# cczls1991/DL_Biomass

Measured on NVIDIA B200. Metric: train tree-clouds/sec @10k pts, higher is better.
Workload: dtype bf16

## Files before the change

### dl_biomass_b200/_lib.py

```python
from __future__ import annotations

import ctypes
import os
import shutil
import subprocess

_HERE = os.path.dirname(os.path.abspath(__file__))
LIB_PATH = os.path.join(_HERE, "libb2pn.so")
CSRC = os.path.join(_HERE, "csrc")

_lib = None
ABI_VERSION = 7

_vp, _i32, _i64, _f32, _f64 = ctypes.c_void_p, ctypes.c_int32, ctypes.c_int64, ctypes.c_float, ctypes.c_double

class Mlp3(ctypes.Structure):
    _fields_ = [("c", ctypes.c_int32 * 4), ("act", ctypes.c_int32), ("eps", ctypes.c_float),
                ("momentum", ctypes.c_float), ("w", _vp * 3), ("b", _vp * 3), ("gamma", _vp * 2),
                ("beta", _vp * 2), ("running_mean", _vp * 2), ("running_var", _vp * 2),
                ("num_batches_tracked", _vp * 2)]


class SaArgs(ctypes.Structure):
    _fields_ = [("precision", ctypes.c_int32), ("training", ctypes.c_int32), ("seg_mode", ctypes.c_int32),
                ("K", ctypes.c_int32), ("n_src", ctypes.c_int64), ("n_dst", ctypes.c_int64),
                ("c_in", ctypes.c_int32), ("x_dtype", ctypes.c_int32), ("x", _vp), ("pos_src", _vp),
                ("pos_dst", _vp), ("nbr", _vp), ("cnt", _vp), ("batch", _vp), ("mlp", Mlp3), ("out", _vp),
                ("arg", _vp), ("h1", _vp), ("h2", _vp), ("bn", _vp), ("workspace", _vp),
                ("workspace_bytes", ctypes.c_int64), ("rgrp", _vp), ("row_src", _vp), ("num_rows", _vp),
                ("row_capacity", ctypes.c_int64), ("row_valid", _vp), ("a1", _vp), ("a2", _vp), ("g1", _vp),
                ("g1_ready", ctypes.c_int32), ("sm_limit", ctypes.c_int32), ("deterministic", ctypes.c_int32),
                ("out_bf16", _vp)]


class FpsOptions(ctypes.Structure):
    _fields_ = [("cluster", ctypes.c_int32), ("threads", ctypes.c_int32), ("seed", ctypes.c_uint64), ("rng_state", _vp)]


class SaGrads(ctypes.Structure):
    _fields_ = [("grad_out", _vp), ("grad_w", _vp * 3), ("grad_b", _vp * 3), ("grad_gamma", _vp * 2),
                ("grad_beta", _vp * 2), ("grad_x", _vp)]

class AugmentCloud(ctypes.Structure):
    _fields_ = [("src_off", ctypes.c_int64), ("out_off", ctypes.c_int64), ("uid", ctypes.c_uint64),
                ("n_src", ctypes.c_int32), ("n_keep", ctypes.c_int32), ("n_dup", ctypes.c_int32),
                ("noise_sd", ctypes.c_float), ("cos_a", ctypes.c_float), ("sin_a", ctypes.c_float)]

# ... 81 lines not shown
```

### dl_biomass_b200/csrc/sa_chain.cuh

```cuda
#pragma once

namespace b2pn {
namespace tc {

constexpr int CH_ROWS = 64;
constexpr int CH_SLOTS = 2;
constexpr int CH_EPI_WARPS = 8;
constexpr int CH_EPI_THREADS = CH_EPI_WARPS * 32;
constexpr int CH_LOAD_THREADS = 128;
constexpr int CH_MMA_WARP = CH_SLOTS * CH_EPI_WARPS;
constexpr int CH_THREADS = CH_SLOTS * CH_EPI_THREADS + CH_SLOTS * 32 + CH_SLOTS * CH_LOAD_THREADS;
constexpr int CH_CHUNK_BYTES = CH_ROWS * LINE_BYTES;
constexpr int CH_TMEM_PER_SLOT = 256;

struct ChainParams {
    const uint8_t *w_img[3];
    int w_bytes[3];
    int k_img;
    int k1c, c1c, c2c;
    int c1, c2, c3;
    int mt3;
    int64_t rows;
    const int64_t *rows_dev;
    const float *bias[3];
// ... 288 lines not shown
                        }
                    }
                }
            }
            tc_fence_before();
            __syncwarp();
            if (lane == 0) mbar_arrive(&b[CB_D3_FREE]);
        }
    }
    tc_fence_before();
    __syncthreads();
    if (warp == CH_MMA_WARP) tmem_dealloc<512>(tmem_base);
}

constexpr int CT_THREADS = CH_SLOTS * CH_EPI_THREADS + CH_SLOTS * 32 + CH_SLOTS * 32;
enum { TB_IN_FULL = 0, TB_IN_FREE, TB_DA_FULL, TB_XA_FULL, TB_DB_FULL, TB_DB_FREE, TB_PER_SLOT };

struct ChainTrainParams {
    const uint8_t *w_img[2];
    int w_bytes[2];
    int k_in;
    int kc_in, kc_mid;
    int c_a, c_b;
    int mt_b;
    int64_t rows;
    const int64_t *rows_dev;
    int64_t ld;
    const float *bias_a, *mean_a, *rstd_a, *gamma_a, *beta_a;
    int dup_a;
    int act;
    __half *z_out, *a_out;
    double *partial;
    int cpad;
    const float *bias_b;
    float *out;
    int32_t *arg;
    __half *out16;
    const uint32_t *rgrp;
};

template <int PASS, int KCI_, int NKSL_, int KCM_, int MTB_>
__global__ void __launch_bounds__(CT_THREADS, 1)
    tc_chain_train_kernel(const ChainTrainParams p, const __grid_constant__ TmaMap map_in, const __grid_constant__ TmaMap map_z,
                          const __grid_constant__ TmaMap map_a)
{
    static_assert(PASS == 2 || PASS == 3, "PASS 2: layer 1 + statistics of layer 2; PASS 3: layer 2 + layer 3 + max");
    const int kc_in = KCI_ >= 0 ? KCI_ : p.kc_in;
    const int kc_mid = KCM_ >= 0 ? KCM_ : p.kc_mid;
    const int mt_b = MTB_ >= 0 ? MTB_ : p.mt_b;
    const int nks_last = NKSL_ >= 0 ? NKSL_ : ((p.k_in - (p.kc_in - 1) * KC) >= KC ? 4 : (p.k_in - (p.kc_in - 1) * KC + 15) / 16);
    extern __shared__ uint8_t smem_raw[];
    uint8_t *smem = reinterpret_cast<uint8_t *>((reinterpret_cast<uintptr_t>(smem_raw) + 1023) & ~(uintptr_t)1023);
    uint8_t *Wa = smem, *Wb = Wa + p.w_bytes[0];
    uint8_t *slots = Wb + p.w_bytes[1];
    const int in_bytes = kc_in * CH_CHUNK_BYTES, x_bytes = kc_mid * CH_CHUNK_BYTES;
    const int slot_bytes = in_bytes + 2 * x_bytes;
    uint64_t *bars = reinterpret_cast<uint64_t *>(slots + CH_SLOTS * slot_bytes);
    uint64_t *w_full = bars + CH_SLOTS * TB_PER_SLOT;
    uint32_t *tmem_holder = reinterpret_cast<uint32_t *>(w_full + 1);

    const int tid = threadIdx.x, warp = tid >> 5, lane = tid & 31;
    const int64_t rows = p.rows_dev ? *p.rows_dev : p.rows;
    const int64_t num_tiles = ((rows + 127) / 128) * 2;

    if (tid == 0) {
        for (int s = 0; s < CH_SLOTS; ++s) {
            uint64_t *b = bars + s * TB_PER_SLOT;
            mbar_init(&b[TB_IN_FULL], 1);
            mbar_init(&b[TB_IN_FREE], 1);
            mbar_init(&b[TB_DA_FULL], 1);
            mbar_init(&b[TB_XA_FULL], 1);
            mbar_init(&b[TB_DB_FULL], 1);
            mbar_init(&b[TB_DB_FREE], CH_EPI_WARPS);
        }
        mbar_init(w_full, 1);
        fence_barrier_init();
    }
    if (warp == CH_MMA_WARP) tmem_alloc<512>(tmem_holder);
    tc_fence_before();
    __syncthreads();
    tc_fence_after();
    const uint32_t tmem_base = *tmem_holder;
    auto tile_of = [&](int64_t it, int s) { return (it * (int64_t)gridDim.x + blockIdx.x) * CH_SLOTS + s; };
    unsigned leader;
    asm volatile("{\n\t.reg .pred p;\n\telect.sync _|p, 0xffffffff;\n\tselp.u32 %0, 1, 0, p;\n\t}" : "=r"(leader));

    if (warp >= CH_MMA_WARP + CH_SLOTS) {
        const int s = warp - (CH_MMA_WARP + CH_SLOTS);
        if (s < CH_SLOTS && leader) {
            uint64_t *b = bars + s * TB_PER_SLOT;
            uint8_t *IN = slots + s * slot_bytes;
            for (int64_t it = 0;; ++it) {
                const int64_t tile = tile_of(it, s);
                if (tile >= num_tiles) break;
                mbar_wait(&b[TB_IN_FREE], (uint32_t)(it & 1) ^ 1u);
                mbar_expect_tx(&b[TB_IN_FULL], (unsigned)in_bytes);
                for (int kc = 0; kc < kc_in; ++kc)
                    tma_load_2d(IN + kc * CH_CHUNK_BYTES, &map_in, (int)(tile * CH_ROWS), kc * KC, &b[TB_IN_FULL]);
                mbar_arrive(&b[TB_IN_FULL]);
            }
        }
    } else if (warp >= CH_MMA_WARP) {
        const int s = warp - CH_MMA_WARP;
        if (s == 0 && leader) {
            mbar_expect_tx(w_full, (unsigned)(p.w_bytes[0] + p.w_bytes[1]));
            for (int l = 0; l < 2; ++l) {
                uint8_t *dst = l == 0 ? Wa : Wb;
                for (int off = 0; off < p.w_bytes[l]; off += 16384) bulk_g2s(dst + off, p.w_img[l] + off, 16384u, w_full);
            }
            mbar_arrive(w_full);
        }
        __syncwarp();
        mbar_wait(w_full, 0);
        const uint32_t idesc_mn = idesc_16(128, CH_ROWS, false, true, FMT_F16, FMT_F16);
        uint64_t *b = bars + s * TB_PER_SLOT;
        uint8_t *IN = slots + s * slot_bytes;
        const uint64_t dwa = smem_desc_sw128(smem_u32(Wa), 16, ATOM_BYTES);
        const uint64_t dwb = smem_desc_sw128(smem_u32(Wb), 16, ATOM_BYTES);
        const uint64_t din = smem_desc_sw128(smem_u32(IN), 64 * LINE_BYTES, ATOM_BYTES);
        const uint64_t dx = smem_desc_sw128(smem_u32(IN + in_bytes), 64 * LINE_BYTES, ATOM_BYTES);
        constexpr uint64_t A_KS = 32 >> 4, A_CHUNK = (128 * LINE_BYTES) >> 4, B_KS_MN = (16 * LINE_BYTES) >> 4,
                           B_CHUNK = CH_CHUNK_BYTES >> 4;
        const uint32_t da = tmem_base + s * CH_TMEM_PER_SLOT, db = da + 64;
        for (int64_t it = 0;; ++it) {
            if (tile_of(it, s) >= num_tiles) break;
            const uint32_t ph = (uint32_t)(it & 1);
            mbar_wait(&b[TB_IN_FULL], ph);
            tc_fence_after();
            if (leader) {
#pragma unroll
                for (int kc = 0; kc < (KCI_ >= 0 ? KCI_ : 3); ++kc) {
                    if (kc < kc_in) {
#pragma unroll
                        for (int ks = 0; ks < 4; ++ks)
                            if (kc + 1 < kc_in || ks < nks_last)
                                umma_bf16(da, dwa + kc * A_CHUNK + ks * A_KS, din + kc * B_CHUNK + ks * B_KS_MN, idesc_mn, (kc | ks) != 0);
                    }
                }
                umma_commit(&b[TB_IN_FREE]);
                umma_commit(&b[TB_DA_FULL]);
            }
            __syncwarp();
            mbar_wait(&b[TB_XA_FULL], ph);
            mbar_wait(&b[TB_DB_FREE], ph ^ 1u);
            tc_fence_after();
            if (leader) {
#pragma unroll
                for (int mt = 0; mt < (MTB_ >= 0 ? MTB_ : 2); ++mt) {
                    if (mt < mt_b) {
#pragma unroll
                        for (int kc = 0; kc < (KCM_ >= 0 ? KCM_ : 2); ++kc) {
                            if (kc < kc_mid) {
#pragma unroll
                                for (int ks = 0; ks < 4; ++ks)
                                    umma_bf16(db + mt * 64, dwb + (uint64_t)(kc * mt_b + mt) * A_CHUNK + ks * A_KS,
                                              dx + kc * B_CHUNK + ks * B_KS_MN, idesc_mn, (kc | ks) != 0);
                            }
                        }
                    }
                }
                umma_commit(&b[TB_DB_FULL]);
            }
            __syncwarp();
        }
    } else {
        const int s = warp / CH_EPI_WARPS, w8 = warp % CH_EPI_WARPS;
        const int q = w8 & 3, half = w8 >> 2;
        uint64_t *b = bars + s * TB_PER_SLOT;
        uint8_t *X = slots + s * slot_bytes + in_bytes;
        const int ch = q * 32 + lane;
        const uint32_t lane_addr = ((uint32_t)(q * 32)) << 16;
        const uint32_t da = tmem_base + lane_addr + s * CH_TMEM_PER_SLOT, db = da + 64;
        const bool dup = (KCM_ == 1 || KCM_ < 0) && p.dup_a != 0;
        const int cha = dup ? (q & 1) * 32 + lane : ch;
        const int col16 = half * 2 + (q >> 1);
        float sc = 0.f, sh = 0.f, ga = 0.f, be = 0.f;
        if (cha < p.c_a) {
            sc = p.rstd_a[cha];
            sh = (p.bias_a[cha] - p.mean_a[cha]) * sc;
            ga = p.gamma_a[cha];
            be = p.beta_a[cha];
        }
        const bool relu = p.act == B2PN_ACT_RELU;
        const int chb = (PASS == 3 && mt_b == 2 ? half * 128 : 0) + ch;
        const bool epb = PASS == 2 || mt_b == 2 || half == 0;
        const float bb = (PASS == 3 && epb && chb < p.c_b) ? p.bias_b[chb] : 0.f;
        uint8_t *xline = X + (cha >> 6) * CH_CHUNK_BYTES + (cha & 63) * LINE_BYTES;
        const int sw = cha & 7;
// ... 8 lines not shown
            const int64_t tile = tile_of(it, s);
            if (tile >= num_tiles) break;
            const uint32_t ph = (uint32_t)(it & 1);
            const int64_t row0 = tile * CH_ROWS;
            unsigned dsc[8] = {nx0.x, nx0.y, nx0.z, nx0.w, nx1.x, nx1.y, nx1.z, nx1.w};
#pragma unroll
            for (int g = 0; g < 8; ++g) {
                const int64_t gi = tile * (CH_ROWS / 8) + g;
                if (gi * 8 >= rows || gi_none(dsc[g])) dsc[g] = GI_NONE;
            }
            if (tile_of(it + 1, s) < num_tiles) {
                const uint4 *t = reinterpret_cast<const uint4 *>(p.rgrp + tile_of(it + 1, s) * (CH_ROWS / 8));
                nx0 = __ldg(t);
                nx1 = __ldg(t + 1);
            }
            mbar_wait(&b[TB_DA_FULL], ph);
            tc_fence_after();
            if (w8 == 0 && lane == 0) bulk_wait_read_all();
            asm volatile("bar.sync %0, %1;" ::"r"(1 + s), "n"(CH_EPI_THREADS) : "memory");
            if (dup) {
                unsigned nv2 = 0u;
#pragma unroll
                for (int g = 0; g < 8; ++g)
                    if ((g >> 1) == col16) nv2 |= (unsigned)gi_nv(dsc[g]) << (4 * (g & 1));
                float v[16];
                tmem_ld16(da + col16 * 16, v);
#pragma unroll
                for (int j = 0; j < 2; ++j) {
                    const int nv = (int)((nv2 >> (4 * j)) & 15u);
                    float f[8], g[8];
#pragma unroll
                    for (int e = 0; e < 8; ++e) f[e] = fmaf(v[8 * j + e], sc, sh);
                    const uint4 zq = pack8h(f);
                    unpack8h(zq, f);
#pragma unroll
                    for (int e = 0; e < 8; ++e) {
                        float y = fmaf(f[e], ga, be);
                        if (relu) y = fmaxf(y, 0.f);
                        g[e] = e < nv ? y : 0.f;
                    }
                    const int off = ((col16 * 2 + j) ^ sw) << 4;
                    *reinterpret_cast<uint4 *>(xline + x_bytes + off) = zq;
                    *reinterpret_cast<uint4 *>(xline + off) = pack8h(g);
                }
            } else if (ch - lane < p.c_a) {
                float v[32];
                tmem_ld32(da + half * 32, v);
#pragma unroll
                for (int j = 0; j < 4; ++j) {
                    const int nv = gi_nv(half == 0 ? dsc[j] : dsc[4 + j]);
                    float f[8], g[8];
#pragma unroll
                    for (int e = 0; e < 8; ++e) f[e] = fmaf(v[8 * j + e], sc, sh);
                    const uint4 zq = pack8h(f);
                    unpack8h(zq, f);
#pragma unroll
                    for (int e = 0; e < 8; ++e) {
                        float y = fmaf(f[e], ga, be);
                        if (relu) y = fmaxf(y, 0.f);
                        g[e] = e < nv ? y : 0.f;
                    }
                    const int off = ((half * 4 + j) ^ sw) << 4;
                    *reinterpret_cast<uint4 *>(xline + x_bytes + off) = zq;
                    *reinterpret_cast<uint4 *>(xline + off) = pack8h(g);
                }
            }
            fence_proxy_async_smem();
            tc_fence_before();
            asm volatile("bar.sync %0, %1;" ::"r"(1 + s), "n"(CH_EPI_THREADS) : "memory");
            if (w8 == 0 && lane == 0) {
                for (int kc = 0; kc < kc_mid; ++kc) {
                    tma_store_2d(&map_z, X + x_bytes + kc * CH_CHUNK_BYTES, (int)row0, kc * KC);
                    tma_store_2d(&map_a, X + kc * CH_CHUNK_BYTES, (int)row0, kc * KC);
                }
                bulk_commit_group();
                mbar_arrive(&b[TB_XA_FULL]);
            }
            mbar_wait(&b[TB_DB_FULL], ph);
            tc_fence_after();
            if (PASS == 2) {
                if (ch - lane < p.c_b) {
                    float v[32];
                    tmem_ld32(db + half * 32, v);
                    float sm = 0.f, qm = 0.f;
#pragma unroll
                    for (int j = 0; j < 32; ++j) {
                        sm += v[j];
                        qm = fmaf(v[j], v[j], qm);
                    }
                    S += (double)sm;
                    Q += (double)qm;
                }
            } else if (epb && chb - lane < p.c_b) {
                const uint32_t dcol = db + (mt_b == 2 ? half * 64 : 0);
                float best = -INFINITY;
                int bk = -1;
#pragma unroll 1
                for (int cc = 0; cc < 2; ++cc) {
                    float v[32];
                    tmem_ld32(dcol + cc * 32, v);
#pragma unroll
                    for (int gg = 0; gg < 4; ++gg) {
                        const unsigned inf = cc == 0 ? dsc[gg] : dsc[4 + gg];
                        if (gi_none(inf)) continue;
                        const int s0 = gi_slot0(inf), nv = gi_nv(inf);
                        if (s0 == 0) {
// ... 11 lines not shown
                        if (gi_last(inf) && chb < p.c_b) {
                            const int64_t m = gi_seg(inf);
                            const float o = bk >= 0 ? best : 0.f;
                            p.out[m * p.c_b + chb] = o;
                            p.arg[m * p.c_b + chb] = bk;
                            if (p.out16) p.out16[m * p.c_b + chb] = __float2half_rn(o);
                        }
                    }
                }
            }
            tc_fence_before();
            __syncwarp();
            if (lane == 0) mbar_arrive(&b[TB_DB_FREE]);
        }
        if (w8 == 0 && lane == 0) bulk_wait_all();
        if (PASS == 2 && ch < p.c_b) {
            double *pt = p.partial + ((int64_t)blockIdx.x * 4 + s * 2 + half) * 2 * p.cpad;
            pt[ch] = S;
            pt[p.cpad + ch] = Q;
        }
    }
    tc_fence_before();
    __syncthreads();
    if (warp == CH_MMA_WARP) tmem_dealloc<512>(tmem_base);
}

static int chain_train_smem_bytes(const ChainTrainParams &p)
{
    return p.w_bytes[0] + p.w_bytes[1] + CH_SLOTS * (p.kc_in + 2 * p.kc_mid) * CH_CHUNK_BYTES + 256 + 1024;
}

static bool chain_shapes_ok(const b2pn_sa_args &a, int k_lines, int c1, int c2, int c3)
{
    return a.seg_mode == B2PN_SEG_SLOTS && c1 % 64 == 0 && c2 % 64 == 0 && c1 <= 128 && c2 <= 128 && c3 <= 256 &&
           k_lines <= 3 * KC;
}

static int chain_smem_bytes(const ChainParams &p)
{
    const int x_bytes = (p.c1c > p.c2c ? p.c1c : p.c2c) * CH_CHUNK_BYTES;
    return p.w_bytes[0] + p.w_bytes[1] + p.w_bytes[2] + CH_SLOTS * (p.k1c * CH_CHUNK_BYTES + x_bytes) + 256 + 1024;
}

}
// ... 2 lines not shown
```

### dl_biomass_b200/csrc/sa_tc.cu

```cuda
#include <cuda.h>
#include <math.h>

#include "tc_common.cuh"

namespace b2pn {
namespace tc {

constexpr int R = 128;
constexpr int KC = 64;
constexpr int NUM_EPI = 256;
constexpr int NUM_LOAD = 128;
constexpr int LOAD_GROUPS = 2;
constexpr int MMA_WARP = (NUM_EPI + LOAD_GROUPS * NUM_LOAD) / 32;
constexpr int NT = NUM_EPI + LOAD_GROUPS * NUM_LOAD + 32;
constexpr int NT_TMA = 2 * NUM_EPI + 64;
constexpr int PROD_WARP_TMA = MMA_WARP + 1;
constexpr int NT_WIDE = 2 * NUM_EPI + 32 + NUM_LOAD;
constexpr int B_BYTES = R * LINE_BYTES;

constexpr unsigned GI_NONE = 0x00ffffffu;
__device__ __forceinline__ int gi_seg(unsigned b) { return (int)(b & 0xffffffu); }
__device__ __forceinline__ bool gi_none(unsigned b) { return (b & 0xffffffu) == 0xffffffu; }
__device__ __forceinline__ int gi_slot0(unsigned b) { return (int)((b >> 24) & 7u) << 3; }
__device__ __forceinline__ int gi_nv(unsigned b) { return (int)((b >> 27) & 15u); }
// ... 1992 lines not shown
    template <class T>
    T *take(int64_t n)
    {
        T *r = base ? (T *)(base + off) : nullptr;
        off = align_up(off + n * (int64_t)sizeof(T), 1024);
        return r;
    }
};

struct ShapesTC {
    int64_t rows, tiles, ld;
    int c0, c1, c2, c3, cmax, cpad, k1;
    InCols cols;
    int ctas;
    bool deterministic;
};
static ShapesTC shapes_tc(const b2pn_sa_args &a)
{
    ShapesTC s;
    s.rows = a.seg_mode == B2PN_SEG_CLOUDS ? a.n_src : a.row_capacity;
    s.tiles = (s.rows + R - 1) / R;
    s.ld = s.tiles * R;
    s.c0 = a.mlp.c[0];
    s.c1 = a.mlp.c[1];
    s.c2 = a.mlp.c[2];
    s.c3 = a.mlp.c[3];
    s.cmax = s.c1 > s.c2 ? s.c1 : s.c2;
    s.cols = InCols{a.c_in, a.x_dtype == B2PN_X_F32 ? 1 : 0};
    s.k1 = s.cols.k_img();
    int mx = s.cmax > s.c3 ? s.cmax : s.c3;
    mx = mx > s.k1 + 1 ? mx : s.k1 + 1;
    s.cpad = (int)align_up(mx, 128);
    s.ctas = cta_budget(a);
    s.deterministic = a.deterministic != 0;
    return s;
}

constexpr int MAX_GX = 160;

int sa_eval_fused_bf16(const b2pn_sa_args &a)
{
    if (a.mlp.c[0] != a.c_in + 3) return 0;
    const ShapesTC s = shapes_tc(a);
    return !a.training && chain_shapes_ok(a, s.k1, s.c1, s.c2, s.c3) ? 1 : 0;
}

static int check_args_tc(const b2pn_sa_args &a)
{
    if (a.n_src < 0 || a.n_dst < 0 || a.c_in < 0) return B2PN_EINVAL;
    if (a.mlp.c[0] != a.c_in + 3 || a.mlp.c[1] <= 0 || a.mlp.c[2] <= 0 || a.mlp.c[3] <= 0) return B2PN_EINVAL;
    if (a.mlp.act != B2PN_ACT_NONE && a.mlp.act != B2PN_ACT_RELU) return B2PN_ENOTSUP;
    if (a.x_dtype != B2PN_X_F32 && a.x_dtype != B2PN_X_BF16) return B2PN_EINVAL;
    if (a.seg_mode == B2PN_SEG_SLOTS) {
        if (a.K <= 0) return B2PN_EINVAL;
        if (a.K > 64) return B2PN_ENOTSUP;
        if (a.n_dst > 0 && (!a.nbr || !a.cnt || !a.pos_dst)) return B2PN_EINVAL;
        if (a.n_dst > 0 && (!a.rgrp || !a.row_src || !a.num_rows)) return B2PN_EINVAL;
        if (a.n_dst > 0 && a.row_capacity < b2pn_pack_rows_capacity(a.n_dst, a.K)) return B2PN_EINVAL;
    } else if (a.seg_mode == B2PN_SEG_CLOUDS) {
        if (a.n_src > 0 && !a.batch) return B2PN_EINVAL;
    } else {
        return B2PN_EINVAL;
    }
    if (a.n_src > 0 && (!a.pos_src || (a.c_in > 0 && !a.x))) return B2PN_EINVAL;
    for (int l = 0; l < 3; ++l)
        if (!a.mlp.w[l] || !a.mlp.b[l]) return B2PN_EINVAL;
    for (int l = 0; l < 2; ++l)
// ... 129 lines not shown
    B2PN_LAUNCH_CHECK();
    return B2PN_OK;
}

static void launch_bn_fwd_finalize(const b2pn_sa_args &a, const ShapesTC &s, int l, const double *partial, int nparts,
                                   const CountArg &count, cudaStream_t st)
{
    const int C = l == 0 ? s.c1 : s.c2;
    bn_fwd_finalize_tc_kernel<<<(C + 3) / 4, 128, 0, st>>>(partial, nparts, C, s.cpad, count, a.training, a.mlp.b[l], a.mlp.gamma[l],
                                                           a.mlp.beta[l], a.mlp.running_mean[l], a.mlp.running_var[l],
                                                           a.mlp.num_batches_tracked[l], a.mlp.eps, a.mlp.momentum,
                                                           a.bn + l * 4 * s.cmax, s.cmax);
    note_launch();
}

static int chain_grid(const ShapesTC &s, int64_t tiles64)
{
    const int64_t need = (tiles64 + CH_SLOTS - 1) / CH_SLOTS;
    return need < s.ctas ? (int)need : s.ctas;
}

template <auto KERN, class... Args>
static int launch_chain(int gx, int threads, int smem, cudaStream_t st, const Args &...args)
{
    static SmemAttrSlot slot = {};
    cudaError_t e = ensure_dynamic_smem(KERN, smem, slot);
    if (e != cudaSuccess) return (int)e;
    KERN<<<gx, threads, smem, st>>>(args...);
    note_launch();
    e = cudaPeekAtLastError();
    return e == cudaSuccess ? 0 : (int)e;
}

int sa_forward_bf16(const b2pn_sa_args &a, cudaStream_t st)
{
    int rc = check_args_tc(a);
    if (rc) return rc;
    const ShapesTC s = shapes_tc(a);
    if (a.n_dst == 0) return B2PN_OK;
    if (a.workspace_bytes < sa_workspace_bytes_bf16(a, 0) || !a.workspace) return B2PN_EINVAL;
    WsTC ws(a.workspace);
    FwdWsTC f = carve_fwd_tc(a, s, ws);
    const RowMapTC rm = rowmap_tc(a, s);
    const RowsArg ra = rowsarg_tc(a, s);
    __nv_bfloat16 *z1 = (__nv_bfloat16 *)a.h1, *z2 = (__nv_bfloat16 *)a.h2;
    float *bn1 = a.bn, *bn2 = a.bn + 4 * s.cmax;
// ... 55 lines not shown
    TmaMap map_g1 = kNoMap;
    TmaFeatLoader tl1;
    if (use_g1 && s.rows > 0) {
        if (!a.g1_ready) launch_gather_l1(a, s, st);
        if ((rc = make_tma_feature_major(&map_g1, a.g1, s.k1 + 1, s.ld))) return rc;
    }
    const int ns1 = use_g1 ? 4 : 2;
    if (train && s.rows > 0) {
        StatsEpTC<1> e1 = {s.c1, f.partial, s.cpad, ns1};
        StatsEpTC<2> e2 = {s.c1, f.partial, s.cpad, ns1};
        rc = use_g1 ? launch_by_mt(f.pk[0], ra, tl1, e1, e2, st, map_g1) : launch_by_mt(f.pk[0], ra, gl, e1, e2, st);
        if (rc) return rc;
    }
    launch_bn_fwd_finalize(a, s, 0, f.partial, ns1 * grid_x_for(f.pk[0], s.tiles, s.ctas), count, st);
    if (train_chain) {
        const int gx = chain_grid(s, s.tiles * 2);
        TmaMap mz1, ma1, mz2, ma2;
        if ((rc = make_tma_feature_major(&mz1, z1, s.c1, s.ld)) || (rc = make_tma_feature_major(&ma1, a.a1, s.c1, s.ld)) ||
            (rc = make_tma_feature_major(&mz2, z2, s.c2, s.ld)) || (rc = make_tma_feature_major(&ma2, a.a2, s.c2, s.ld)))
            return rc;
        ChainTrainParams p2 = {};
        p2.w_img[0] = f.pk[0].img; p2.w_bytes[0] = (int)f.pk[0].bytes;
        p2.w_img[1] = f.pk[1].img; p2.w_bytes[1] = (int)f.pk[1].bytes;
        p2.k_in = s.k1; p2.kc_in = f.pk[0].num_kc; p2.kc_mid = f.pk[1].num_kc;
        p2.c_a = s.c1; p2.c_b = s.c2; p2.mt_b = 1; p2.dup_a = s.c1 == 64;
        p2.rows = ra.cap; p2.rows_dev = ra.dev; p2.ld = s.ld;
        p2.bias_a = a.mlp.b[0]; p2.mean_a = bn1; p2.rstd_a = bn1 + s.cmax; p2.gamma_a = a.mlp.gamma[0]; p2.beta_a = a.mlp.beta[0];
        p2.act = a.mlp.act; p2.z_out = (__half *)z1; p2.a_out = (__half *)a.a1;
        p2.partial = f.partial; p2.cpad = s.cpad; p2.rgrp = a.rgrp;
        const int smem2 = chain_train_smem_bytes(p2);
        const int nks1 = (s.k1 - (p2.kc_in - 1) * KC) >= KC ? 4 : (s.k1 - (p2.kc_in - 1) * KC + 15) / 16;
        if (p2.kc_in == 1 && nks1 == 1 && p2.kc_mid == 1)
            rc = launch_chain<tc_chain_train_kernel<2, 1, 1, 1, 1>>(gx, CT_THREADS, smem2, st, p2, map_g1, mz1, ma1);
        else if (p2.kc_in == 3 && nks1 == 1 && p2.kc_mid == 2)
            rc = launch_chain<tc_chain_train_kernel<2, 3, 1, 2, 1>>(gx, CT_THREADS, smem2, st, p2, map_g1, mz1, ma1);
        else
            rc = launch_chain<tc_chain_train_kernel<2, -1, -1, -1, -1>>(gx, CT_THREADS, smem2, st, p2, map_g1, mz1, ma1);
        if (rc) return rc;
        launch_bn_fwd_finalize(a, s, 1, f.partial, 4 * gx, count, st);
        TmaMap map_in3;
        if ((rc = make_tma_feature_major(&map_in3, a.a1, s.c1, s.ld))) return rc;
        ChainTrainParams p3 = {};
        p3.w_img[0] = f.pk[1].img; p3.w_bytes[0] = (int)f.pk[1].bytes;
        p3.w_img[1] = f.pk[2].img; p3.w_bytes[1] = (int)f.pk[2].bytes;
        p3.k_in = s.c1; p3.kc_in = f.pk[1].num_kc; p3.kc_mid = f.pk[2].num_kc;
        p3.c_a = s.c2; p3.c_b = s.c3; p3.mt_b = f.pk[2].MT; p3.dup_a = s.c2 == 64;
        p3.rows = ra.cap; p3.rows_dev = ra.dev; p3.ld = s.ld;
        p3.bias_a = a.mlp.b[1]; p3.mean_a = bn2; p3.rstd_a = bn2 + s.cmax; p3.gamma_a = a.mlp.gamma[1]; p3.beta_a = a.mlp.beta[1];
        p3.act = a.mlp.act; p3.z_out = (__half *)z2; p3.a_out = (__half *)a.a2;
        p3.bias_b = a.mlp.b[2]; p3.out = a.out; p3.arg = a.arg; p3.out16 = (__half *)a.out_bf16; p3.rgrp = a.rgrp;
        const int smem3 = chain_train_smem_bytes(p3);
        if (p3.kc_in == 1 && p3.kc_mid == 1 && p3.mt_b == 1)
            return launch_chain<tc_chain_train_kernel<3, 1, 4, 1, 1>>(gx, CT_THREADS, smem3, st, p3, map_in3, mz2, ma2);
        if (p3.kc_in == 2 && p3.kc_mid == 2 && p3.mt_b == 2)
            return launch_chain<tc_chain_train_kernel<3, 2, 4, 2, 2>>(gx, CT_THREADS, smem3, st, p3, map_in3, mz2, ma2);
        return launch_chain<tc_chain_train_kernel<3, -1, -1, -1, -1>>(gx, CT_THREADS, smem3, st, p3, map_in3, mz2, ma2);
    }
    if (s.rows > 0) {
        NormStoreEpTC e = {s.c1, a.mlp.b[0], bn1, bn1 + s.cmax, a.mlp.gamma[0], a.mlp.beta[0], a.mlp.act, rm};
        TmaMap mz, ma;
        if ((rc = make_tma_feature_major(&mz, z1, s.c1, s.ld, 32))) return rc;
        if ((rc = make_tma_feature_major(&ma, a.a1, s.c1, s.ld, 32))) return rc;
        rc = use_g1 ? launch_by_mt(f.pk[0], ra, tl1, e, e, st, map_g1, mz, ma) : launch_by_mt(f.pk[0], ra, gl, e, e, st, kNoMap, mz, ma);
        if (rc) return rc;
    }
    TmaFeatLoader l2, l3;
    TmaMap map_a1, map_a2;
    if ((rc = make_tma_feature_major(&map_a1, a.a1, s.c1, s.ld))) return rc;
    if ((rc = make_tma_feature_major(&map_a2, a.a2, s.c2, s.ld))) return rc;
    if (train && s.rows > 0) {
        StatsEpTC<1> e1 = {s.c2, f.partial, s.cpad, 4};
// ... 238 lines not shown
```

### dl_biomass_b200/sa.py

```python
from __future__ import annotations

import ctypes
import threading
from contextlib import contextmanager
from typing import List, Optional, Sequence

import torch

from . import _lib
from .optim import fresh_alias, grad_dst

PREC_F32, PREC_BF16 = 0, 1

H16 = torch.float16
SEG_SLOTS, SEG_CLOUDS = 0, 1
ACT_NONE, ACT_RELU = 0, 1

_vp = ctypes.c_void_p


Mlp3, SaArgs, SaGrads = _lib.Mlp3, _lib.SaArgs, _lib.SaGrads


def _dp(t: Optional[torch.Tensor]):
    return None if t is None else t.data_ptr()


class LaunchOptions:
    __slots__ = ("sm_limit", "deterministic")

    def __init__(self, sm_limit: int = 0, deterministic: int = 0):
        self.sm_limit, self.deterministic = int(sm_limit), int(deterministic)


_tls = threading.local()


def current_options() -> LaunchOptions:
    h = getattr(_tls, "holder", None)
    if h is None:
        h = _tls.holder = LaunchOptions()
    return h


def launch_options():
    h = current_options()
    return h.sm_limit, h.deterministic
# ... 1 lines not shown

def set_sm_limit(n: int) -> None:
    if n < 0:
        raise ValueError("sm_limit must be >= 0")
    current_options().sm_limit = int(n)


def set_deterministic(on: bool) -> bool:
    h = current_options()
    prev = bool(h.deterministic)
    h.deterministic = 1 if on else 0
    return prev


@contextmanager
def options(sm_limit: Optional[int] = None, deterministic: Optional[bool] = None):
    h = current_options()
    prev = (h.sm_limit, h.deterministic)
    try:
        if sm_limit is not None:
            set_sm_limit(sm_limit)
        if deterministic is not None:
            set_deterministic(deterministic)
        yield h
    finally:
        h.sm_limit, h.deterministic = prev


def act_code(act) -> int:
    if act is None:
        return ACT_NONE
    name = act if isinstance(act, str) else type(act).__name__
    if name.lower() == "relu":
        return ACT_RELU
    raise NotImplementedError(
        f"activation {act!r}: the B200 kernels implement ReLU (the only activation the reference trains with, "
        f"/root/reference/main.py:45) and None")


def _fill_args(a: SaArgs, *, precision, training, seg_mode, K, n_src, n_dst, c_in, x, pos_src, pos_dst, nbr, cnt,
               batch, chans, act, eps, momentum, ws, bs, gammas, betas, rmeans, rvars, nbts, out, arg, h1, h2, bn,
               rowmap=None, acts=None, out_bf16=None, holder=None):
    a.precision, a.training, a.seg_mode, a.K = precision, int(training), seg_mode, K
    h = holder if holder is not None else current_options()
    a.sm_limit, a.deterministic = h.sm_limit, h.deterministic
    a.out_bf16 = _dp(out_bf16)
    a.n_src, a.n_dst, a.c_in = n_src, n_dst, c_in
    a.x_dtype = 1 if (x is not None and x.dtype == H16) else 0
    a.x, a.pos_src, a.pos_dst = _dp(x), _dp(pos_src), _dp(pos_dst)
    a.nbr, a.cnt, a.batch = _dp(nbr), _dp(cnt), _dp(batch)
    m = a.mlp
    for i in range(4):
        m.c[i] = chans[i]
    m.act, m.eps, m.momentum = act, eps, momentum
    for i in range(3):
        m.w[i], m.b[i] = _dp(ws[i]), _dp(bs[i])
    for i in range(2):
        m.gamma[i], m.beta[i] = _dp(gammas[i]), _dp(betas[i])
        m.running_mean[i], m.running_var[i] = _dp(rmeans[i]), _dp(rvars[i])
        m.num_batches_tracked[i] = _dp(nbts[i])
# ... 262 lines not shown
```

### include/b2pn.h

```cpp
#ifndef B2PN_H_
#define B2PN_H_

#include <stdint.h>

#ifdef __cplusplus
extern "C" {
#endif

#define B2PN_ABI_VERSION 7
#define B2PN_OK 0
#define B2PN_EINVAL (-1)
#define B2PN_ENOTSUP (-2)

typedef void *b2pn_stream_t;

int b2pn_abi_version(void);
const char *b2pn_error_string(int code);
int64_t b2pn_launch_count(void);

int64_t b2pn_fps_num_samples(int64_t n, float ratio);

typedef struct b2pn_fps_options {
    int32_t cluster;
    int32_t threads;
// ... 65 lines not shown
    int32_t *arg;
    void *h1, *h2;
    float *bn;
    void *workspace;
    int64_t workspace_bytes;
    const uint32_t *rgrp;
    const int32_t *row_src;
    const int64_t *num_rows;
    int64_t row_capacity;
    const void *row_valid;
    void *a1, *a2;
    void *g1;
    int32_t g1_ready;
    int32_t sm_limit;
    int32_t deterministic;
    void *out_bf16;
} b2pn_sa_args;

typedef struct b2pn_sa_grads {
    const float *grad_out;
    float *grad_w[3], *grad_b[3];
    float *grad_gamma[2], *grad_beta[2];
    float *grad_x;
} b2pn_sa_grads;

int64_t b2pn_sa_workspace_bytes(const b2pn_sa_args *args, int32_t backward);
int b2pn_sa_forward(const b2pn_sa_args *args, b2pn_stream_t stream);
int b2pn_sa_eval_fused(const b2pn_sa_args *args);
int b2pn_sa_gather_rows(const b2pn_sa_args *args, b2pn_stream_t stream);
int b2pn_sa_backward(const b2pn_sa_args *args, const b2pn_sa_grads *grads, b2pn_stream_t stream);
// ... 65 lines not shown
```

Baseline: 6052.

## Add four-slot variant of training chain kernel for single-M-tile second GEMM

Adds a SLOTS=4 template variant of the fused training chain kernel. Each slot gets a quarter of TMEM and 4 epilogue warps. The MMA warp takes over input TMA prefetch from the dedicated producer warp, and the dup-64 BN statistics are reduced through shared memory. The host picks four slots when the second GEMM has one M tile and the shared-memory budget fits, with an option to force two slots. The aim is more tiles in flight per CTA to hide latency. The cost is fewer epilogue warps per tile and extra serial work per epilogue thread.

```diff
diff --git a/dl_biomass_b200/_lib.py b/dl_biomass_b200/_lib.py
--- a/dl_biomass_b200/_lib.py
+++ b/dl_biomass_b200/_lib.py
@@ -10,7 +10,7 @@
 CSRC = os.path.join(_HERE, "csrc")
 
 _lib = None
-ABI_VERSION = 7
+ABI_VERSION = 8
 
 _vp, _i32, _i64, _f32, _f64 = ctypes.c_void_p, ctypes.c_int32, ctypes.c_int64, ctypes.c_float, ctypes.c_double
 
@@ -30,7 +30,7 @@
                 ("workspace_bytes", ctypes.c_int64), ("rgrp", _vp), ("row_src", _vp), ("num_rows", _vp),
                 ("row_capacity", ctypes.c_int64), ("row_valid", _vp), ("a1", _vp), ("a2", _vp), ("g1", _vp),
                 ("g1_ready", ctypes.c_int32), ("sm_limit", ctypes.c_int32), ("deterministic", ctypes.c_int32),
-                ("out_bf16", _vp)]
+                ("chain_slots", ctypes.c_int32), ("out_bf16", _vp)]
 
 
 class FpsOptions(ctypes.Structure):
diff --git a/dl_biomass_b200/csrc/sa_chain.cuh b/dl_biomass_b200/csrc/sa_chain.cuh
--- a/dl_biomass_b200/csrc/sa_chain.cuh
+++ b/dl_biomass_b200/csrc/sa_chain.cuh
@@ -326,6 +326,7 @@
 }
 
 constexpr int CT_THREADS = CH_SLOTS * CH_EPI_THREADS + CH_SLOTS * 32 + CH_SLOTS * 32;
+static_assert(CT_THREADS == 16 * 32 + 4 * 32, "four slots: 16 epilogue warps + 4 MMA / producer warps");
 enum { TB_IN_FULL = 0, TB_IN_FREE, TB_DA_FULL, TB_XA_FULL, TB_DB_FULL, TB_DB_FREE, TB_PER_SLOT };
 
 struct ChainTrainParams {
@@ -340,6 +341,7 @@
     int64_t ld;
     const float *bias_a, *mean_a, *rstd_a, *gamma_a, *beta_a;
     int dup_a;
+    int dup_b;
     int act;
     __half *z_out, *a_out;
     double *partial;
@@ -351,15 +353,17 @@
     const uint32_t *rgrp;
 };
 
-template <int PASS, int KCI_, int NKSL_, int KCM_, int MTB_>
+template <int PASS, int KCI_, int NKSL_, int KCM_, int MTB_, int SLOTS>
 __global__ void __launch_bounds__(CT_THREADS, 1)
     tc_chain_train_kernel(const ChainTrainParams p, const __grid_constant__ TmaMap map_in, const __grid_constant__ TmaMap map_z,
                           const __grid_constant__ TmaMap map_a)
 {
     static_assert(PASS == 2 || PASS == 3, "PASS 2: layer 1 + statistics of layer 2; PASS 3: layer 2 + layer 3 + max");
+    static_assert(SLOTS == 2 || (SLOTS == 4 && MTB_ <= 1), "four slots hold one M tile of the second GEMM");
+    constexpr int EPI_WARPS = 16 / SLOTS, EPI_THREADS = EPI_WARPS * 32, TMEM_PER_SLOT = 512 / SLOTS;
     const int kc_in = KCI_ >= 0 ? KCI_ : p.kc_in;
     const int kc_mid = KCM_ >= 0 ? KCM_ : p.kc_mid;
-    const int mt_b = MTB_ >= 0 ? MTB_ : p.mt_b;
+    const int mt_b = SLOTS == 4 ? 1 : (MTB_ >= 0 ? MTB_ : p.mt_b);
     const int nks_last = NKSL_ >= 0 ? NKSL_ : ((p.k_in - (p.kc_in - 1) * KC) >= KC ? 4 : (p.k_in - (p.kc_in - 1) * KC + 15) / 16);
     extern __shared__ uint8_t smem_raw[];
     uint8_t *smem = reinterpret_cast<uint8_t *>((reinterpret_cast<uintptr_t>(smem_raw) + 1023) & ~(uintptr_t)1023);
@@ -367,8 +371,8 @@
     uint8_t *slots = Wb + p.w_bytes[1];
     const int in_bytes = kc_in * CH_CHUNK_BYTES, x_bytes = kc_mid * CH_CHUNK_BYTES;
     const int slot_bytes = in_bytes + 2 * x_bytes;
-    uint64_t *bars = reinterpret_cast<uint64_t *>(slots + CH_SLOTS * slot_bytes);
-    uint64_t *w_full = bars + CH_SLOTS * TB_PER_SLOT;
+    uint64_t *bars = reinterpret_cast<uint64_t *>(slots + SLOTS * slot_bytes);
+    uint64_t *w_full = bars + SLOTS * TB_PER_SLOT;
     uint32_t *tmem_holder = reinterpret_cast<uint32_t *>(w_full + 1);
 
     const int tid = threadIdx.x, warp = tid >> 5, lane = tid & 31;
@@ -376,14 +380,14 @@
     const int64_t num_tiles = ((rows + 127) / 128) * 2;
 
     if (tid == 0) {
-        for (int s = 0; s < CH_SLOTS; ++s) {
+        for (int s = 0; s < SLOTS; ++s) {
             uint64_t *b = bars + s * TB_PER_SLOT;
             mbar_init(&b[TB_IN_FULL], 1);
             mbar_init(&b[TB_IN_FREE], 1);
             mbar_init(&b[TB_DA_FULL], 1);
             mbar_init(&b[TB_XA_FULL], 1);
             mbar_init(&b[TB_DB_FULL], 1);
-            mbar_init(&b[TB_DB_FREE], CH_EPI_WARPS);
+            mbar_init(&b[TB_DB_FREE], EPI_WARPS);
         }
         mbar_init(w_full, 1);
         fence_barrier_init();
@@ -393,13 +397,13 @@
     __syncthreads();
     tc_fence_after();
     const uint32_t tmem_base = *tmem_holder;
-    auto tile_of = [&](int64_t it, int s) { return (it * (int64_t)gridDim.x + blockIdx.x) * CH_SLOTS + s; };
+    auto tile_of = [&](int64_t it, int s) { return (it * (int64_t)gridDim.x + blockIdx.x) * SLOTS + s; };
     unsigned leader;
     asm volatile("{\n\t.reg .pred p;\n\telect.sync _|p, 0xffffffff;\n\tselp.u32 %0, 1, 0, p;\n\t}" : "=r"(leader));
 
-    if (warp >= CH_MMA_WARP + CH_SLOTS) {
-        const int s = warp - (CH_MMA_WARP + CH_SLOTS);
-        if (s < CH_SLOTS && leader) {
+    if (SLOTS == 2 && warp >= CH_MMA_WARP + SLOTS) {
+        const int s = warp - (CH_MMA_WARP + SLOTS);
+        if (s < SLOTS && leader) {
             uint64_t *b = bars + s * TB_PER_SLOT;
             uint8_t *IN = slots + s * slot_bytes;
             for (int64_t it = 0;; ++it) {
@@ -414,6 +418,15 @@
         }
     } else if (warp >= CH_MMA_WARP) {
         const int s = warp - CH_MMA_WARP;
+        uint64_t *b = bars + s * TB_PER_SLOT;
+        uint8_t *IN = slots + s * slot_bytes;
+        auto load_in = [&](int64_t tile) {
+            mbar_expect_tx(&b[TB_IN_FULL], (unsigned)in_bytes);
+            for (int kc = 0; kc < kc_in; ++kc)
+                tma_load_2d(IN + kc * CH_CHUNK_BYTES, &map_in, (int)(tile * CH_ROWS), kc * KC, &b[TB_IN_FULL]);
+            mbar_arrive(&b[TB_IN_FULL]);
+        };
+        if (SLOTS == 4 && leader && tile_of(0, s) < num_tiles) load_in(tile_of(0, s));
         if (s == 0 && leader) {
             mbar_expect_tx(w_full, (unsigned)(p.w_bytes[0] + p.w_bytes[1]));
             for (int l = 0; l < 2; ++l) {
@@ -425,15 +438,13 @@
         __syncwarp();
         mbar_wait(w_full, 0);
         const uint32_t idesc_mn = idesc_16(128, CH_ROWS, false, true, FMT_F16, FMT_F16);
-        uint64_t *b = bars + s * TB_PER_SLOT;
-        uint8_t *IN = slots + s * slot_bytes;
         const uint64_t dwa = smem_desc_sw128(smem_u32(Wa), 16, ATOM_BYTES);
         const uint64_t dwb = smem_desc_sw128(smem_u32(Wb), 16, ATOM_BYTES);
         const uint64_t din = smem_desc_sw128(smem_u32(IN), 64 * LINE_BYTES, ATOM_BYTES);
         const uint64_t dx = smem_desc_sw128(smem_u32(IN + in_bytes), 64 * LINE_BYTES, ATOM_BYTES);
         constexpr uint64_t A_KS = 32 >> 4, A_CHUNK = (128 * LINE_BYTES) >> 4, B_KS_MN = (16 * LINE_BYTES) >> 4,
                            B_CHUNK = CH_CHUNK_BYTES >> 4;
-        const uint32_t da = tmem_base + s * CH_TMEM_PER_SLOT, db = da + 64;
+        const uint32_t da = tmem_base + s * TMEM_PER_SLOT, db = da + 64;
         for (int64_t it = 0;; ++it) {
             if (tile_of(it, s) >= num_tiles) break;
             const uint32_t ph = (uint32_t)(it & 1);
@@ -453,6 +464,11 @@
                 umma_commit(&b[TB_DA_FULL]);
             }
             __syncwarp();
+            if (SLOTS == 4 && tile_of(it + 1, s) < num_tiles) {
+                mbar_wait(&b[TB_IN_FREE], ph);
+                if (leader) load_in(tile_of(it + 1, s));
+                __syncwarp();
+            }
             mbar_wait(&b[TB_XA_FULL], ph);
             mbar_wait(&b[TB_DB_FREE], ph ^ 1u);
             tc_fence_after();
@@ -476,14 +492,15 @@
             __syncwarp();
         }
     } else {
-        const int s = warp / CH_EPI_WARPS, w8 = warp % CH_EPI_WARPS;
+        const int s = warp / EPI_WARPS, w8 = warp % EPI_WARPS;
         const int q = w8 & 3, half = w8 >> 2;
         uint64_t *b = bars + s * TB_PER_SLOT;
         uint8_t *X = slots + s * slot_bytes + in_bytes;
         const int ch = q * 32 + lane;
         const uint32_t lane_addr = ((uint32_t)(q * 32)) << 16;
-        const uint32_t da = tmem_base + lane_addr + s * CH_TMEM_PER_SLOT, db = da + 64;
+        const uint32_t da = tmem_base + lane_addr + s * TMEM_PER_SLOT, db = da + 64;
         const bool dup = (KCM_ == 1 || KCM_ < 0) && p.dup_a != 0;
+        const bool dup_b = SLOTS == 4 && PASS == 2 && p.dup_b != 0;
         const int cha = dup ? (q & 1) * 32 + lane : ch;
         const int col16 = half * 2 + (q >> 1);
         float sc = 0.f, sh = 0.f, ga = 0.f, be = 0.f;
@@ -522,11 +539,40 @@
                 nx0 = __ldg(t);
                 nx1 = __ldg(t + 1);
             }
+            auto norm32 = [&](int hh) {
+                float v[32];
+                tmem_ld32(da + hh * 32, v);
+#pragma unroll
+                for (int j = 0; j < 4; ++j) {
+                    const int nv = gi_nv(hh == 0 ? dsc[j] : dsc[4 + j]);
+                    float f[8], g[8];
+#pragma unroll
+                    for (int e = 0; e < 8; ++e) f[e] = fmaf(v[8 * j + e], sc, sh);
+                    const uint4 zq = pack8h(f);
+                    unpack8h(zq, f);
+#pragma unroll
+                    for (int e = 0; e < 8; ++e) {
+                        float y = fmaf(f[e], ga, be);
+                        if (relu) y = fmaxf(y, 0.f);
+                        g[e] = e < nv ? y : 0.f;
+                    }
+                    const int off = ((hh * 4 + j) ^ sw) << 4;
+                    *reinterpret_cast<uint4 *>(xline + x_bytes + off) = zq;
+                    *reinterpret_cast<uint4 *>(xline + off) = pack8h(g);
+                }
+            };
             mbar_wait(&b[TB_DA_FULL], ph);
             tc_fence_after();
             if (w8 == 0 && lane == 0) bulk_wait_read_all();
-            asm volatile("bar.sync %0, %1;" ::"r"(1 + s), "n"(CH_EPI_THREADS) : "memory");
-            if (dup) {
+            asm volatile("bar.sync %0, %1;" ::"r"(1 + s), "n"(EPI_THREADS) : "memory");
+            if (SLOTS == 4) {
+                if (dup) {
+                    norm32(q >> 1);
+                } else if (ch - lane < p.c_a) {
+#pragma unroll 1
+                    for (int hh = 0; hh < 2; ++hh) norm32(hh);
+                }
+            } else if (dup) {
                 unsigned nv2 = 0u;
 #pragma unroll
                 for (int g = 0; g < 8; ++g)
@@ -552,30 +598,11 @@
                     *reinterpret_cast<uint4 *>(xline + off) = pack8h(g);
                 }
             } else if (ch - lane < p.c_a) {
-                float v[32];
-                tmem_ld32(da + half * 32, v);
-#pragma unroll
-                for (int j = 0; j < 4; ++j) {
-                    const int nv = gi_nv(half == 0 ? dsc[j] : dsc[4 + j]);
-                    float f[8], g[8];
-#pragma unroll
-                    for (int e = 0; e < 8; ++e) f[e] = fmaf(v[8 * j + e], sc, sh);
-                    const uint4 zq = pack8h(f);
-                    unpack8h(zq, f);
-#pragma unroll
-                    for (int e = 0; e < 8; ++e) {
-                        float y = fmaf(f[e], ga, be);
-                        if (relu) y = fmaxf(y, 0.f);
-                        g[e] = e < nv ? y : 0.f;
-                    }
-                    const int off = ((half * 4 + j) ^ sw) << 4;
-                    *reinterpret_cast<uint4 *>(xline + x_bytes + off) = zq;
-                    *reinterpret_cast<uint4 *>(xline + off) = pack8h(g);
-                }
+                norm32(half);
             }
             fence_proxy_async_smem();
             tc_fence_before();
-            asm volatile("bar.sync %0, %1;" ::"r"(1 + s), "n"(CH_EPI_THREADS) : "memory");
+            asm volatile("bar.sync %0, %1;" ::"r"(1 + s), "n"(EPI_THREADS) : "memory");
             if (w8 == 0 && lane == 0) {
                 for (int kc = 0; kc < kc_mid; ++kc) {
                     tma_store_2d(&map_z, X + x_bytes + kc * CH_CHUNK_BYTES, (int)row0, kc * KC);
@@ -587,9 +614,9 @@
             mbar_wait(&b[TB_DB_FULL], ph);
             tc_fence_after();
             if (PASS == 2) {
-                if (ch - lane < p.c_b) {
+                auto stats32 = [&](int hh) {
                     float v[32];
-                    tmem_ld32(db + half * 32, v);
+                    tmem_ld32(db + hh * 32, v);
                     float sm = 0.f, qm = 0.f;
 #pragma unroll
                     for (int j = 0; j < 32; ++j) {
@@ -598,6 +625,16 @@
                     }
                     S += (double)sm;
                     Q += (double)qm;
+                };
+                if (dup_b) {
+                    stats32(q >> 1);
+                } else if (ch - lane < p.c_b) {
+                    if (SLOTS == 4) {
+#pragma unroll 1
+                        for (int hh = 0; hh < 2; ++hh) stats32(hh);
+                    } else {
+                        stats32(half);
+                    }
                 }
             } else if (epb && chb - lane < p.c_b) {
                 const uint32_t dcol = db + (mt_b == 2 ? half * 64 : 0);
@@ -639,10 +676,31 @@
             if (lane == 0) mbar_arrive(&b[TB_DB_FREE]);
         }
         if (w8 == 0 && lane == 0) bulk_wait_all();
-        if (PASS == 2 && ch < p.c_b) {
+        if (PASS == 2 && SLOTS == 2 && ch < p.c_b) {
             double *pt = p.partial + ((int64_t)blockIdx.x * 4 + s * 2 + half) * 2 * p.cpad;
             pt[ch] = S;
             pt[p.cpad + ch] = Q;
+        }
+        if (PASS == 2 && SLOTS == 4) {
+            int c = ch;
+            if (dup_b) {
+                double *red = reinterpret_cast<double *>(slots + s * slot_bytes);
+                c = (q & 1) * 32 + lane;
+                if (q >= 2) {
+                    red[c] = S;
+                    red[64 + c] = Q;
+                }
+                asm volatile("bar.sync %0, %1;" ::"r"(1 + s), "n"(EPI_THREADS) : "memory");
+                if (q < 2) {
+                    S += red[c];
+                    Q += red[64 + c];
+                }
+            }
+            if ((!dup_b || q < 2) && c < p.c_b) {
+                double *pt = p.partial + ((int64_t)blockIdx.x * 4 + s) * 2 * p.cpad;
+                pt[c] = S;
+                pt[p.cpad + c] = Q;
+            }
         }
     }
     tc_fence_before();
@@ -650,9 +708,9 @@
     if (warp == CH_MMA_WARP) tmem_dealloc<512>(tmem_base);
 }
 
-static int chain_train_smem_bytes(const ChainTrainParams &p)
+static int chain_train_smem_bytes(const ChainTrainParams &p, int slots)
 {
-    return p.w_bytes[0] + p.w_bytes[1] + CH_SLOTS * (p.kc_in + 2 * p.kc_mid) * CH_CHUNK_BYTES + 256 + 1024;
+    return p.w_bytes[0] + p.w_bytes[1] + slots * (p.kc_in + 2 * p.kc_mid) * CH_CHUNK_BYTES + 256 + 1024;
 }
 
 static bool chain_shapes_ok(const b2pn_sa_args &a, int k_lines, int c1, int c2, int c3)
diff --git a/dl_biomass_b200/csrc/sa_tc.cu b/dl_biomass_b200/csrc/sa_tc.cu
--- a/dl_biomass_b200/csrc/sa_tc.cu
+++ b/dl_biomass_b200/csrc/sa_tc.cu
@@ -2030,6 +2030,7 @@
     InCols cols;
     int ctas;
     bool deterministic;
+    int chain_slots;
 };
 static ShapesTC shapes_tc(const b2pn_sa_args &a)
 {
@@ -2049,6 +2050,7 @@
     s.cpad = (int)align_up(mx, 128);
     s.ctas = cta_budget(a);
     s.deterministic = a.deterministic != 0;
+    s.chain_slots = a.chain_slots;
     return s;
 }
 
@@ -2067,6 +2069,7 @@
     if (a.mlp.c[0] != a.c_in + 3 || a.mlp.c[1] <= 0 || a.mlp.c[2] <= 0 || a.mlp.c[3] <= 0) return B2PN_EINVAL;
     if (a.mlp.act != B2PN_ACT_NONE && a.mlp.act != B2PN_ACT_RELU) return B2PN_ENOTSUP;
     if (a.x_dtype != B2PN_X_F32 && a.x_dtype != B2PN_X_BF16) return B2PN_EINVAL;
+    if (a.chain_slots != 0 && a.chain_slots != 2) return B2PN_EINVAL;
     if (a.seg_mode == B2PN_SEG_SLOTS) {
         if (a.K <= 0) return B2PN_EINVAL;
         if (a.K > 64) return B2PN_ENOTSUP;
@@ -2226,9 +2229,9 @@
     note_launch();
 }
 
-static int chain_grid(const ShapesTC &s, int64_t tiles64)
-{
-    const int64_t need = (tiles64 + CH_SLOTS - 1) / CH_SLOTS;
+static int chain_grid(const ShapesTC &s, int64_t tiles64, int slots = CH_SLOTS)
+{
+    const int64_t need = (tiles64 + slots - 1) / slots;
     return need < s.ctas ? (int)need : s.ctas;
 }
 
@@ -2242,6 +2245,25 @@
     note_launch();
     e = cudaPeekAtLastError();
     return e == cudaSuccess ? 0 : (int)e;
+}
+
+static int chain_train_slots(const ShapesTC &s, const ChainTrainParams &p)
+{
+    constexpr int SMEM_MAX = 227 * 1024;
+    return s.chain_slots != 2 && p.mt_b == 1 && chain_train_smem_bytes(p, 4) <= SMEM_MAX ? 4 : 2;
+}
+
+template <int PASS, int KCI, int NKSL, int KCM, int MTB, bool FOUR>
+static int launch_chain_train(int slots, int gx, cudaStream_t st, const ChainTrainParams &p, const TmaMap &map_in,
+                              const TmaMap &map_z, const TmaMap &map_a)
+{
+    if constexpr (FOUR) {
+        if (slots == 4)
+            return launch_chain<tc_chain_train_kernel<PASS, KCI, NKSL, KCM, MTB, 4>>(gx, CT_THREADS, chain_train_smem_bytes(p, 4),
+                                                                                     st, p, map_in, map_z, map_a);
+    }
+    return launch_chain<tc_chain_train_kernel<PASS, KCI, NKSL, KCM, MTB, 2>>(gx, CT_THREADS, chain_train_smem_bytes(p, 2), st,
+                                                                             p, map_in, map_z, map_a);
 }
 
 int sa_forward_bf16(const b2pn_sa_args &a, cudaStream_t st)
@@ -2327,7 +2349,6 @@
     }
     launch_bn_fwd_finalize(a, s, 0, f.partial, ns1 * grid_x_for(f.pk[0], s.tiles, s.ctas), count, st);
     if (train_chain) {
-        const int gx = chain_grid(s, s.tiles * 2);
         TmaMap mz1, ma1, mz2, ma2;
         if ((rc = make_tma_feature_major(&mz1, z1, s.c1, s.ld)) || (rc = make_tma_feature_major(&ma1, a.a1, s.c1, s.ld)) ||
             (rc = make_tma_feature_major(&mz2, z2, s.c2, s.ld)) || (rc = make_tma_feature_major(&ma2, a.a2, s.c2, s.ld)))
@@ -2336,21 +2357,22 @@
         p2.w_img[0] = f.pk[0].img; p2.w_bytes[0] = (int)f.pk[0].bytes;
         p2.w_img[1] = f.pk[1].img; p2.w_bytes[1] = (int)f.pk[1].bytes;
         p2.k_in = s.k1; p2.kc_in = f.pk[0].num_kc; p2.kc_mid = f.pk[1].num_kc;
-        p2.c_a = s.c1; p2.c_b = s.c2; p2.mt_b = 1; p2.dup_a = s.c1 == 64;
+        p2.c_a = s.c1; p2.c_b = s.c2; p2.mt_b = 1; p2.dup_a = s.c1 == 64; p2.dup_b = s.c2 == 64;
         p2.rows = ra.cap; p2.rows_dev = ra.dev; p2.ld = s.ld;
         p2.bias_a = a.mlp.b[0]; p2.mean_a = bn1; p2.rstd_a = bn1 + s.cmax; p2.gamma_a = a.mlp.gamma[0]; p2.beta_a = a.mlp.beta[0];
         p2.act = a.mlp.act; p2.z_out = (__half *)z1; p2.a_out = (__half *)a.a1;
         p2.partial = f.partial; p2.cpad = s.cpad; p2.rgrp = a.rgrp;
-        const int smem2 = chain_train_smem_bytes(p2);
+        const int slots2 = chain_train_slots(s, p2);
+        const int gx2 = chain_grid(s, s.tiles * 2, slots2);
         const int nks1 = (s.k1 - (p2.kc_in - 1) * KC) >= KC ? 4 : (s.k1 - (p2.kc_in - 1) * KC + 15) / 16;
         if (p2.kc_in == 1 && nks1 == 1 && p2.kc_mid == 1)
-            rc = launch_chain<tc_chain_train_kernel<2, 1, 1, 1, 1>>(gx, CT_THREADS, smem2, st, p2, map_g1, mz1, ma1);
+            rc = launch_chain_train<2, 1, 1, 1, 1, true>(slots2, gx2, st, p2, map_g1, mz1, ma1);
         else if (p2.kc_in == 3 && nks1 == 1 && p2.kc_mid == 2)
-            rc = launch_chain<tc_chain_train_kernel<2, 3, 1, 2, 1>>(gx, CT_THREADS, smem2, st, p2, map_g1, mz1, ma1);
+            rc = launch_chain_train<2, 3, 1, 2, 1, false>(slots2, gx2, st, p2, map_g1, mz1, ma1);
         else
-            rc = launch_chain<tc_chain_train_kernel<2, -1, -1, -1, -1>>(gx, CT_THREADS, smem2, st, p2, map_g1, mz1, ma1);
+            rc = launch_chain_train<2, -1, -1, -1, -1, true>(slots2, gx2, st, p2, map_g1, mz1, ma1);
         if (rc) return rc;
-        launch_bn_fwd_finalize(a, s, 1, f.partial, 4 * gx, count, st);
+        launch_bn_fwd_finalize(a, s, 1, f.partial, 4 * gx2, count, st);
         TmaMap map_in3;
         if ((rc = make_tma_feature_major(&map_in3, a.a1, s.c1, s.ld))) return rc;
         ChainTrainParams p3 = {};
@@ -2362,12 +2384,13 @@
         p3.bias_a = a.mlp.b[1]; p3.mean_a = bn2; p3.rstd_a = bn2 + s.cmax; p3.gamma_a = a.mlp.gamma[1]; p3.beta_a = a.mlp.beta[1];
         p3.act = a.mlp.act; p3.z_out = (__half *)z2; p3.a_out = (__half *)a.a2;
         p3.bias_b = a.mlp.b[2]; p3.out = a.out; p3.arg = a.arg; p3.out16 = (__half *)a.out_bf16; p3.rgrp = a.rgrp;
-        const int smem3 = chain_train_smem_bytes(p3);
+        const int slots3 = chain_train_slots(s, p3);
+        const int gx3 = chain_grid(s, s.tiles * 2, slots3);
         if (p3.kc_in == 1 && p3.kc_mid == 1 && p3.mt_b == 1)
-            return launch_chain<tc_chain_train_kernel<3, 1, 4, 1, 1>>(gx, CT_THREADS, smem3, st, p3, map_in3, mz2, ma2);
+            return launch_chain_train<3, 1, 4, 1, 1, true>(slots3, gx3, st, p3, map_in3, mz2, ma2);
         if (p3.kc_in == 2 && p3.kc_mid == 2 && p3.mt_b == 2)
-            return launch_chain<tc_chain_train_kernel<3, 2, 4, 2, 2>>(gx, CT_THREADS, smem3, st, p3, map_in3, mz2, ma2);
-        return launch_chain<tc_chain_train_kernel<3, -1, -1, -1, -1>>(gx, CT_THREADS, smem3, st, p3, map_in3, mz2, ma2);
+            return launch_chain_train<3, 2, 4, 2, 2, false>(slots3, gx3, st, p3, map_in3, mz2, ma2);
+        return launch_chain_train<3, -1, -1, -1, -1, true>(slots3, gx3, st, p3, map_in3, mz2, ma2);
     }
     if (s.rows > 0) {
         NormStoreEpTC e = {s.c1, a.mlp.b[0], bn1, bn1 + s.cmax, a.mlp.gamma[0], a.mlp.beta[0], a.mlp.act, rm};
diff --git a/dl_biomass_b200/sa.py b/dl_biomass_b200/sa.py
--- a/dl_biomass_b200/sa.py
+++ b/dl_biomass_b200/sa.py
@@ -27,10 +27,10 @@
 
 
 class LaunchOptions:
-    __slots__ = ("sm_limit", "deterministic")
-
-    def __init__(self, sm_limit: int = 0, deterministic: int = 0):
-        self.sm_limit, self.deterministic = int(sm_limit), int(deterministic)
+    __slots__ = ("sm_limit", "deterministic", "chain_slots")
+
+    def __init__(self, sm_limit: int = 0, deterministic: int = 0, chain_slots: int = 0):
+        self.sm_limit, self.deterministic, self.chain_slots = int(sm_limit), int(deterministic), int(chain_slots)
 
 
 _tls = threading.local()
@@ -62,17 +62,21 @@
 
 
 @contextmanager
-def options(sm_limit: Optional[int] = None, deterministic: Optional[bool] = None):
+def options(sm_limit: Optional[int] = None, deterministic: Optional[bool] = None, chain_slots: Optional[int] = None):
     h = current_options()
-    prev = (h.sm_limit, h.deterministic)
+    prev = (h.sm_limit, h.deterministic, h.chain_slots)
     try:
         if sm_limit is not None:
             set_sm_limit(sm_limit)
         if deterministic is not None:
             set_deterministic(deterministic)
+        if chain_slots is not None:
+            if chain_slots not in (0, 2):
+                raise ValueError("chain_slots must be 0 (from the shape) or 2")
+            h.chain_slots = int(chain_slots)
         yield h
     finally:
-        h.sm_limit, h.deterministic = prev
+        h.sm_limit, h.deterministic, h.chain_slots = prev
 
 
 def act_code(act) -> int:
@@ -91,7 +95,7 @@
                rowmap=None, acts=None, out_bf16=None, holder=None):
     a.precision, a.training, a.seg_mode, a.K = precision, int(training), seg_mode, K
     h = holder if holder is not None else current_options()
-    a.sm_limit, a.deterministic = h.sm_limit, h.deterministic
+    a.sm_limit, a.deterministic, a.chain_slots = h.sm_limit, h.deterministic, h.chain_slots
     a.out_bf16 = _dp(out_bf16)
     a.n_src, a.n_dst, a.c_in = n_src, n_dst, c_in
     a.x_dtype = 1 if (x is not None and x.dtype == H16) else 0
diff --git a/include/b2pn.h b/include/b2pn.h
--- a/include/b2pn.h
+++ b/include/b2pn.h
@@ -7,7 +7,7 @@
 extern "C" {
 #endif
 
-#define B2PN_ABI_VERSION 7
+#define B2PN_ABI_VERSION 8
 #define B2PN_OK 0
 #define B2PN_EINVAL (-1)
 #define B2PN_ENOTSUP (-2)
@@ -103,6 +103,7 @@
     int32_t g1_ready;
     int32_t sm_limit;
     int32_t deterministic;
+    int32_t chain_slots;
     void *out_bf16;
 } b2pn_sa_args;
 
```

Result: faster. 6147 (median of 6 runs) (+1.6%).
